# cp2k/dbcsr

Measured on AMD Instinct MI355X. Metric: block-sparse multiply GFLOP/s (fp64), higher is better.
Workload: dtype f64; 1 GPU; config2_32768_23x23_fill10_fp64; M=32768, c_nblks=2030625, nproducts=29207882, k_passes=1, parallelism=1 GPU

## Files before the change

dbcsr_amd/csrc/mm_choose.h:

```cpp
#ifndef DBCSR_AMD_MM_CHOOSE_H
#define DBCSR_AMD_MM_CHOOSE_H

#include <algorithm>
#include <cstddef>
#include <cstdint>
#include <cstdio>

namespace dbcsr_amd {

#define DBCSR_AMD_HOT_SIZES(X) \
  X(9) X(10) X(11) X(12) X(13) X(14) X(15) X(16) X(17) X(18) X(19) X(20) X(21) X(22) X(23) X(24) X(25) X(26) X(27) X(28) X(29) X(30) X(31) X(32)
#define DBCSR_AMD_DMA_SIZES(X) X(13) X(16) X(23) X(32)
#define DBCSR_AMD_F32_DIRECT_SIZES(X) X(16) X(24) X(32)
#define DBCSR_AMD_MID_SHAPES(X)                                                                             \
  X(6, 8) X(6, 9) X(6, 10) X(6, 11) X(6, 12)                                                                \
  X(7, 9) X(7, 10) X(7, 11) X(7, 12)                                                                        \
  X(8, 6) X(8, 8) X(8, 9) X(8, 10) X(8, 11) X(8, 12)                                                        \
  X(9, 6) X(9, 7) X(9, 8) X(9, 9) X(9, 10) X(9, 11) X(9, 12)                                                \
  X(10, 6) X(10, 7) X(10, 8) X(10, 9) X(10, 10) X(10, 11) X(10, 12)                                         \
  X(11, 6) X(11, 7) X(11, 8) X(11, 9) X(11, 10) X(11, 11) X(11, 12)                                         \
  X(12, 6) X(12, 7) X(12, 8) X(12, 9) X(12, 10) X(12, 11) X(12, 12)

#define DBCSR_AMD_IS_(S_) || s == S_
static inline bool hot_f64_has(int m, int n, int k) { const int s = m; return m == n && m == k && (false DBCSR_AMD_HOT_SIZES(DBCSR_AMD_IS_)); }
// ... 232 lines not shown
  c.variant = (lab.dbg & ~32) ? 1 : lab.hot_variant;
  if (hot_allowed && hot_f64_has(hm, hn, hk)) return pick(Family::f64_hot, per_wave, dbg_flags, "mm_numeric_f64_hot<%d,%d,%d>", hm, hn, hk);
  if (sw.use_pipe == 1 || (sw.use_pipe < 0 && f.nproducts < 6 * nblk && f.nproducts > nblk + nblk / 2)) {
    c.group = sw.pipe_g;
    c.lds_bytes = 4 * wave_bytes + (size_t)lab.lds_pad;
    return pick(Family::f64_pipe, (unsigned)((npos + 4 * (int64_t)c.group - 1) / (4 * (int64_t)c.group)), skip, "mm_numeric_f64_pipe<%d>", c.maxt);
  }
  return pick(Family::f64_lds, lds_grid, dbg_flags, "mm_numeric_f64_lds<%d>", c.maxt);
}

struct SymbolicSizes {
  int nbr = 0, nbk = 0, nbc = 0;
  int64_t a_nblks = 0, b_nblks = 0;
  bool filtering = false, retain = false;
  int forced = 0;
};

struct SymbolicChoice {
  bool sparse_guess = false;
  bool bitmap_rows = false;
  bool grid_kernels = false, rows_kernels = false;
};

static inline SymbolicChoice choose_symbolic_pattern(const SymbolicSizes& s) {
  SymbolicChoice c;
  const double prod_est = (double)s.a_nblks * ((double)s.b_nblks / (double)std::max(s.nbk, 1));
  c.sparse_guess = s.forced == 3 || (s.forced == 0 && s.nbr >= 2048 && prod_est < 0.6 * (double)s.nbr * (double)s.nbc);
  c.bitmap_rows = s.filtering && c.sparse_guess && !s.retain;
  return c;
}

static inline SymbolicChoice choose_symbolic_count(const SymbolicSizes& s, SymbolicChoice c, int64_t c_nblks) {
  const int nJ = (s.nbc + 63) / 64;
  c.grid_kernels = s.filtering || (((int64_t)s.nbr * nJ * 64 <= 256 * std::max<int64_t>(c_nblks, 1)) && s.forced != 1);
  c.rows_kernels = s.forced == 3 || (s.forced == 0 && s.nbr >= 2048 && 10 * c_nblks < 6 * (int64_t)s.nbr * s.nbc);
  if (c.rows_kernels) c.grid_kernels = false;
  return c;
}

static inline void choose_panels(int W, int64_t b_bytes_est, int64_t panel_bytes, int* NP_out, int* PW_out) {
  int NP = (int)std::min<int64_t>((b_bytes_est + panel_bytes - 1) / panel_bytes, (int64_t)W);
  if (NP < 1) NP = 1;
  const int PW = (W + NP - 1) / NP;
  *NP_out = (W + PW - 1) / PW;
  *PW_out = PW;
}

static inline int64_t panel_bytes_of_mb(long long mb) { return (int64_t)std::max<long long>(mb, 1) << 20; }

}
#endif
```

dbcsr_amd/csrc/mm_engine.hip:

```cpp
#include <hip/hip_runtime.h>

#include <cstdio>
#include <cstdlib>
#include <cstring>
#include <algorithm>
#include <new>
#include <vector>

#include "../../include/dbcsr_amd_mm.h"
#include "common.h"
#include "smm_core.h"
#include "mm_types.h"
#include "mm_complex.h"
#include "mm_jit.h"

#include "mm_workspace.h"
#include "mm_symbolic.h"
#include "mm_numeric_f64.h"
#include "mm_numeric_f64_big.h"
#include "mm_numeric_f64_small.h"
#include "mm_mid.h"
#include "mm_numeric_f32.h"
#include "mm_numeric_z64.h"
#include "mm_aux.h"
// ... 23 lines not shown
#include "mm_engine_plan.h"
#ifdef DBCSR_AMD_EXPERIMENTS
#include "mm_engine_lab.h"
#endif


static int build_product_lists(Engine* E, bool reuse, const dbcsr_amd_bcsr* a, const dbcsr_amd_bcsr* b, const dbcsr_amd_bcsr* c_in, dbcsr_amd_bcsr* c_out,
                               hipStream_t st) {
  const int nbr = E->facts.nbr, W = E->W, nbc = b->nblkcols, nJ = (nbc + 63) / 64;
  const int64_t nblk = E->facts.c_nblks;
  const uint32_t* cin_bm = E->have_cin ? E->cin_bm.p : nullptr;
  const int* cin_pre = E->have_cin ? E->cin_pre.p : nullptr;
  if (reuse) {
    ACC_CHECK(hipMemcpyAsync(c_out->col_i, E->plan_c_col_i.p, sizeof(int32_t) * (size_t)nblk, hipMemcpyDeviceToDevice, st));
    ACC_CHECK(hipMemcpyAsync(c_out->blk_p, E->plan_c_blk_p.p, sizeof(int64_t) * (size_t)nblk, hipMemcpyDeviceToDevice, st));
  } else if (E->rows_kernels) {
    if (E->tmp_i32.ensure((size_t)nblk + 1)) return -1;
    ACC_CHECK(hipMemsetAsync(E->tmp_i32.p, 0, sizeof(int) * (size_t)nblk, st));
    hipLaunchKernelGGL(fill_products_rows, grid_for((int64_t)nbr * 64), dim3(256), 0, st, a->row_p, a->col_i, a->blk_p, a->col_blk_size, b->row_p,
                       b->col_i, b->blk_p, E->c_bm.p, E->c_pre.p, c_out->row_p, E->prod_start.p, nbr, W, E->tmp_i32.p, E->entries.p, E->filter);
    hipLaunchKernelGGL(finish_descs_grid, grid_for((int64_t)nbr * nJ * 64), dim3(256), 0, st, c_in->row_p, c_in->blk_p, c_out->row_blk_size,
                       c_out->col_blk_size, cin_bm, cin_pre, E->c_bm.p, E->c_pre.p, c_out->row_p, E->c_blk_p_ws.p, E->prod_start.p,
                       E->prod_cnt.p, nbr, W, nJ, c_out->col_i, c_out->blk_p, E->descs.p);
  } else if (E->grid_kernels) {
    hipLaunchKernelGGL(fill_products_grid, grid_for((int64_t)nbr * nJ * 64), dim3(256), 0, st, a->row_p, a->col_i, a->blk_p, b->row_p,
                       b->blk_p, c_in->row_p, c_in->blk_p, a->row_blk_size, a->col_blk_size, b->col_blk_size, E->b_bm.p, E->b_pre.p,
                       cin_bm, cin_pre, E->c_bm.p, E->c_pre.p, c_out->row_p, E->prod_start.p, E->c_blk_p_ws.p, nbr, nbc, W, nJ, c_out->col_i,
                       c_out->blk_p, E->descs.p, E->entries.p, E->filter);
  } else {
    hipLaunchKernelGGL(fill_products, grid_for((int64_t)nbr * W), dim3(256), 0, st, a->row_p, a->col_i, a->blk_p, b->row_p, b->blk_p,
// ... 244 lines not shown
  if (E->b_bm.ensure((size_t)nbk * W + 1) || E->b_pre.ensure((size_t)nbk * W + 1) || E->c_bm.ensure((size_t)nbr * W + 1) ||
      E->c_pre.ensure((size_t)nbr * W + 1) || E->row_nnz.ensure((size_t)nbr + 1) || E->dev_scalars.ensure(16))
    return -1;
  if (E->have_cin && (E->cin_bm.ensure((size_t)nbr * W + 1) || E->cin_pre.ensure((size_t)nbr * W + 1))) return -1;
  ACC_CHECK(hipMemsetAsync(E->dev_scalars.p, 0, 16 * sizeof(unsigned long long), st));
  {
    static const int init[6] = {0, -0x7fffffff, 0, -0x7fffffff, 0, -0x7fffffff};
    ACC_CHECK(hipMemcpyAsync(E->dev_scalars.p + 4, init, sizeof(init), hipMemcpyHostToDevice, st));
  }
  if (nbr == 0 || nbc == 0) {
    ACC_CHECK(hipMemsetAsync(c_out_row_p, 0, sizeof(int32_t) * ((size_t)nbr + 1), st));
    ACC_CHECK(hipStreamSynchronize(st));
    counts->c_nblks = counts->c_nze = counts->nproducts = counts->flop = 0;
    E->facts.c_nblks = 0;
    E->facts.nproducts = 0;
    E->grid_kernels = E->rows_kernels = false;
    E->facts.cls_mode = false;
    E->sym_bitmap = -1;
    E->sym_NP = E->sym_PW = E->sym_rowp_chunks = 0;
    E->valid = true;
    return 0;
  }
  ACC_CHECK(hipMemsetAsync(E->b_bm.p, 0, sizeof(uint32_t) * (size_t)nbk * W, st));
  if (nbk > 0) {
    hipLaunchKernelGGL(bitmap_from_index, grid_for((int64_t)nbk * 64), dim3(256), 0, st, b->row_p, b->col_i, nbk, W, E->b_bm.p);
    hipLaunchKernelGGL(row_prefix, grid_for((int64_t)nbk * 64), dim3(256), 0, st, E->b_bm.p, nbk, W, E->b_pre.p, (int*)nullptr);
  }
  if (E->have_cin) {
    ACC_CHECK(hipMemsetAsync(E->cin_bm.p, 0, sizeof(uint32_t) * (size_t)nbr * W, st));
    hipLaunchKernelGGL(bitmap_from_index, grid_for((int64_t)nbr * 64), dim3(256), 0, st, c_in->row_p, c_in->col_i, nbr, W,
                       E->cin_bm.p);
// ... 11 lines not shown
    } else if (datatype == dbcsr_type_complex_8) {
      hipLaunchKernelGGL((bcsr_block_norms<z64>), grid_for((int64_t)nbr * sa * 64), dim3(256), 0, st, a->row_p, a->col_i, a->blk_p,
                         static_cast<const z64*>(a->data), a->row_blk_size, a->col_blk_size, nbr, sa, 1.0, E->a_norms.p, (double*)nullptr);
      hipLaunchKernelGGL((bcsr_block_norms<z64>), grid_for((int64_t)nbk * sb * 64), dim3(256), 0, st, b->row_p, b->col_i, b->blk_p,
                         static_cast<const z64*>(b->data), b->row_blk_size, b->col_blk_size, nbk, sb, alpha, E->b_norms.p, (double*)nullptr);
    } else {
      hipLaunchKernelGGL((bcsr_block_norms<float>), grid_for((int64_t)nbr * sa * 64), dim3(256), 0, st, a->row_p, a->col_i, a->blk_p,
                         static_cast<const float*>(a->data), a->row_blk_size, a->col_blk_size, nbr, sa, 1.0, E->a_norms.p, (double*)nullptr);
      hipLaunchKernelGGL((bcsr_block_norms<float>), grid_for((int64_t)nbk * sb * 64), dim3(256), 0, st, b->row_p, b->col_i, b->blk_p,
                         static_cast<const float*>(b->data), b->row_blk_size, b->col_blk_size, nbk, sb, alpha, E->b_norms.p, (double*)nullptr);
    }
    E->filter = FilterArgs{E->a_norms.p, E->b_norms.p, (float)filter_eps};
  }
  SymbolicSizes sizes;
  sizes.nbr = nbr, sizes.nbk = nbk, sizes.nbc = nbc, sizes.a_nblks = a->nblks, sizes.b_nblks = b->nblks;
  sizes.filtering = filtering, sizes.retain = retain_sparsity != 0, sizes.forced = E->force_symbolic;
  SymbolicChoice sym = choose_symbolic_pattern(sizes);
  if (sym.bitmap_rows) {
    if (E->have_cin)
      ACC_CHECK(hipMemcpyAsync(E->c_bm.p, E->cin_bm.p, sizeof(uint32_t) * (size_t)nbr * W, hipMemcpyDeviceToDevice, st));
    else
      ACC_CHECK(hipMemsetAsync(E->c_bm.p, 0, sizeof(uint32_t) * (size_t)nbr * W, st));
    hipLaunchKernelGGL(c_bitmap_rows_filtered, grid_for((int64_t)nbr * 64), dim3(256), 0, st, a->row_p, a->col_i, b->row_p, b->col_i, nbr, W,
                       E->facts.canonical_c, E->filter, E->c_bm.p);
  } else if (filtering)
    hipLaunchKernelGGL(c_bitmap_filtered, grid_for((int64_t)nbr * ((nbc + 63) / 64) * 64), dim3(256), 0, st, a->row_p, a->col_i, b->row_p,
                       E->b_bm.p, E->b_pre.p, E->have_cin ? E->cin_bm.p : (const uint32_t*)nullptr, nbr, nbc, W, (nbc + 63) / 64,
                       retain_sparsity ? 1 : 0, E->facts.canonical_c, E->filter, E->c_bm.p);
  else
    hipLaunchKernelGGL(c_bitmap, grid_for((int64_t)nbr * W), dim3(256), 0, st, a->row_p, a->col_i, E->b_bm.p,
                       E->have_cin ? E->cin_bm.p : (const uint32_t*)nullptr, nbr, W, retain_sparsity ? 1 : 0, E->facts.canonical_c, E->c_bm.p);
// ... 64 lines not shown
  } else {
  hipLaunchKernelGGL(order_count, grid_for(nkeys), dim3(256), 0, st, E->c_pre.p, E->row_nnz.p, nbr, W, PW, NP, NG, RG, E->order_cnt.p);
  if (exclusive_scan<int64_t>(E, E->order_cnt.p, nkeys, E->order_base.p, nullptr, false, st)) return -1;
  hipLaunchKernelGGL(order_len, dim3(1), dim3(1), 0, st, E->order_base.p, c_nblks, NP, NG, dsc + 7);
  }
  if (E->prod_cnt.ensure((size_t)c_nblks + 1) || E->blk_nze.ensure((size_t)c_nblks + 1) || E->prod_start.ensure((size_t)c_nblks + 1) ||
      E->c_blk_p_ws.ensure((size_t)c_nblks + 1))
    return -1;
  const int nJ = (nbc + 63) / 64;
  sym = choose_symbolic_count(sizes, sym, c_nblks);
  E->grid_kernels = sym.grid_kernels;
  E->rows_kernels = sym.rows_kernels;
  E->sym_bitmap = sym.bitmap_rows ? 2 : (filtering ? 1 : 0);
  E->sym_NP = NP, E->sym_PW = PW;
  E->sym_rowp_chunks = (int)(((int64_t)nbr + kScanChunk - 1) / kScanChunk);
  if (E->rows_kernels) {
    ACC_CHECK(hipMemsetAsync(E->prod_cnt.p, 0, sizeof(int) * (size_t)c_nblks, st));
    hipLaunchKernelGGL(block_sizes_rows, grid_for((int64_t)nbr * W), dim3(256), 0, st, E->c_bm.p, E->c_pre.p, c_out_row_p, a->row_blk_size,
                       b->col_blk_size, nbr, W, E->blk_nze.p);
    hipLaunchKernelGGL(count_products_rows, grid_for((int64_t)nbr * 64), dim3(256), 0, st, a->row_p, a->col_i, a->row_blk_size, a->col_blk_size,
                       b->col_blk_size, b->row_p, b->col_i, E->c_bm.p, E->c_pre.p, c_out_row_p, nbr, W, E->prod_cnt.p, E->dev_scalars.p + 3,
                       E->filter);
  } else if (E->grid_kernels)
    hipLaunchKernelGGL(count_products_grid, grid_for((int64_t)nbr * nJ * 64), dim3(256), 0, st, a->row_p, a->col_i, a->row_blk_size,
                       a->col_blk_size, b->col_blk_size, E->b_bm.p, E->c_bm.p, E->c_pre.p, c_out_row_p, nbr, nbc, W, nJ,
                       E->prod_cnt.p, E->blk_nze.p, E->dev_scalars.p + 3, b->row_p, E->b_pre.p, E->filter);
  else
    hipLaunchKernelGGL(count_products, grid_for((int64_t)nbr * W), dim3(256), 0, st, a->row_p, a->col_i, a->row_blk_size,
                       a->col_blk_size, b->col_blk_size, E->b_bm.p, E->c_bm.p, E->c_pre.p, c_out_row_p, nbr, W, E->prod_cnt.p,
                       E->blk_nze.p, E->dev_scalars.p + 3);
  if (exclusive_scan<int64_t>(E, E->prod_cnt.p, c_nblks, E->prod_start.p, dsc + 2, false, st)) return -1;
  if (exclusive_scan<int64_t>(E, E->blk_nze.p, c_nblks, E->c_blk_p_ws.p, dsc + 1, false, st)) return -1;
  ACC_CHECK(hipMemcpyAsync(E->host_scalars, dsc, 8 * sizeof(int64_t), hipMemcpyDeviceToHost, st));
  ACC_CHECK(hipStreamSynchronize(st));
  E->facts.order_len = E->host_scalars[7];
  if (E->facts.cls_mode) {
    for (int c = 0; c < kNumClasses; ++c) {
      E->cls_len[c] = E->cls_host_lens[c];
      E->cls_off[c] = E->cls_host_lens[kNumClasses + c];
    }
    const int64_t total = E->cls_host_lens[2 * kNumClasses];
    E->facts.order_len = total / 8;
    if (E->order.ensure((size_t)total + 64)) return -1;
    if (total > 0) {
      ACC_CHECK(hipMemsetAsync(E->order.p, 0xff, sizeof(int) * ((size_t)total + 64), st));
      hipLaunchKernelGGL(order_fill_cls, grid_for((int64_t)nbr * W), dim3(256), 0, st, E->c_bm.p, E->c_pre.p, c_out_row_p, E->cls_row.p,
// ... 121 lines not shown
```

dbcsr_amd/csrc/mm_engine_env.h:

```cpp
#ifndef DBCSR_AMD_MM_ENGINE_ENV_H
#define DBCSR_AMD_MM_ENGINE_ENV_H

static void engine_read_env(Engine* E) {
  if (const char* k = getenv("DBCSR_AMD_MM_KERNEL")) {
    E->sw.use_lds = strcmp(k, "direct") != 0;
    E->sw.use_pipe = strcmp(k, "pipe") == 0 ? 1 : (strcmp(k, "lds1") == 0 ? 0 : -1);
#ifdef DBCSR_AMD_EXPERIMENTS
    if (strncmp(k, "dma", 3) == 0 && k[3] >= '2' && k[3] <= '4') E->lab.dma_stages = k[3] - '0';
#endif
  }
  if (const char* k = getenv("DBCSR_AMD_MM_PIPE_G")) E->sw.pipe_g = std::max(1, atoi(k));
  if (const char* k = getenv("DBCSR_AMD_MM_CLASSES")) E->sw.use_classes = atoi(k);
  if (const char* k = getenv("DBCSR_AMD_MM_WORK")) E->sw.use_work = atoi(k);
  if (const char* k = getenv("DBCSR_AMD_MM_WG_WAVES")) {
    const int w = atoi(k);
    if (w == 1 || w == 2 || w == 4) E->sw.wg_waves = w;
  }
  if (const char* k = getenv("DBCSR_AMD_MM_PLAN")) E->use_plan = atoi(k);
  if (const char* k = getenv("DBCSR_AMD_MM_HOT")) E->sw.use_hot = atoi(k);
  if (const char* k = getenv("DBCSR_AMD_MM_TINY")) E->sw.use_tiny = atoi(k);
  if (const char* k = getenv("DBCSR_AMD_MM_SMALL")) E->sw.use_small = atoi(k);
  if (const char* k = getenv("DBCSR_AMD_MM_SMALL_G")) E->sw.small_group = std::min(64, std::max(0, atoi(k)));
  if (const char* k = getenv("DBCSR_AMD_MM_F32_DIRECT")) E->sw.f32_direct = atoi(k);
  if (const char* k = getenv("DBCSR_AMD_MM_BIG")) E->sw.use_big = atoi(k);
  if (const char* k = getenv("DBCSR_AMD_MM_MID")) E->sw.use_mid = atoi(k);
  if (const char* k = getenv("DBCSR_AMD_MM_SYMBOLIC")) {
    E->force_symbolic = strcmp(k, "word") == 0 ? 1 : (strcmp(k, "grid") == 0 ? 2 : (strcmp(k, "rows") == 0 ? 3 : 0));
  }
  if (const char* k = getenv("DBCSR_AMD_MM_PANEL_MB")) E->panel_bytes = panel_bytes_of_mb(atoll(k));
#ifdef DBCSR_AMD_EXPERIMENTS
  if (const char* k = getenv("DBCSR_AMD_MM_F32_GROUP")) {
    const int r = atoi(k);
    E->lab.f32_group = (r >= 2 && r <= 4) ? r : (r < 0 ? -1 : 0);
  }
  if (const char* k = getenv("DBCSR_AMD_MM_F64_GROUP")) E->lab.f64_group = atoi(k);
  if (const char* k = getenv("DBCSR_AMD_MM_GROUP_PANEL_MB")) E->ls.group_panel_bytes = panel_bytes_of_mb(atoll(k));
  if (const char* k = getenv("DBCSR_AMD_MM_CLASS_G")) {
    const int g = atoi(k);
    E->lab.class_g = (g == 2 || g == 4 || g == 8) ? g : 1;
  }
  if (const char* k = getenv("DBCSR_AMD_MM_DBG")) E->lab.dbg = atoi(k);
  if (const char* k = getenv("DBCSR_AMD_ALG_COLSUMS")) E->ls.alg_col_variant = atoi(k);
  if (const char* k = getenv("DBCSR_AMD_MULTIVEC_WAVES")) E->ls.multivec_waves = atoi(k);
// ... 28 lines not shown
```

dbcsr_amd/csrc/mm_engine_ops.h:

```cpp
#ifndef DBCSR_AMD_MM_ENGINE_OPS_H
#define DBCSR_AMD_MM_ENGINE_OPS_H

static int init_c_any(void* handle, libsmm_acc_data_t datatype, double beta, double beta_im, const dbcsr_amd_bcsr* c_in, dbcsr_amd_bcsr* c_out,
                      void* stream) {
  Engine* E = static_cast<Engine*>(handle);
  if (E) E->plan_numeric = false;
  if (!E || !E->valid || !c_in || !c_out) {
    fprintf(stderr, "dbcsr_amd_mm_init_c: no valid symbolic phase for this handle\n");
    return -1;
  }
  if (datatype != dbcsr_type_real_8 && datatype != dbcsr_type_real_4 && datatype != dbcsr_type_complex_8) return -10;
  hipStream_t st = stream_of(stream);
  const int nbr = E->facts.nbr, W = E->W;
  const int64_t nblk = E->facts.c_nblks;
  engine_writes_values(E);
  c_out->nblks = nblk;
  if (nblk == 0) return 0;
  if (E->descs.ensure((size_t)nblk + 1)) return -1;
  hipLaunchKernelGGL(emit_index, grid_for((int64_t)nbr * W), dim3(256), 0, st, c_in->row_p, c_in->blk_p, c_out->row_blk_size,
                     c_out->col_blk_size, E->have_cin ? E->cin_bm.p : (const uint32_t*)nullptr,
                     E->have_cin ? E->cin_pre.p : (const int*)nullptr, E->c_bm.p, E->c_pre.p, c_out->row_p, E->c_blk_p_ws.p, nbr, W,
                     c_out->col_i, c_out->blk_p, E->descs.p);
  if (datatype == dbcsr_type_real_8)
    hipLaunchKernelGGL((init_c_blocks<double>), grid_for(nblk * 64), dim3(256), 0, st, E->descs.p, nblk,
// ... 467 lines not shown
const char* dbcsr_amd_mm_last_kernel(void* handle) {
  Engine* E = static_cast<Engine*>(handle);
  return E ? E->last_kernel : "";
}

const char* dbcsr_amd_mm_last_symbolic(void* handle) {
  Engine* E = static_cast<Engine*>(handle);
  if (!E) return "";
  static const char* const bitmap[] = {"none", "plain", "filtered", "rows_filtered"};
  snprintf(E->last_symbolic, sizeof E->last_symbolic, "bitmap=%s count=%s W=%d NP=%d PW=%d classes=%d rowp_chunks=%d plan=%s",
           bitmap[std::min(std::max(E->sym_bitmap, -1), 2) + 1], E->sym_bitmap < 0 ? "none" : (E->rows_kernels ? "rows" : (E->grid_kernels ? "grid" : "word")),
           E->W, E->sym_NP, E->sym_PW, E->facts.cls_mode ? 1 : 0, E->sym_rowp_chunks, E->plan_hit ? "hit" : "miss");
  return E->last_symbolic;
}

int dbcsr_amd_mm_expect_filter(void* handle, double eps) {
  Engine* E = static_cast<Engine*>(handle);
  if (!E || !(eps >= 0.0)) return -1;
  E->drop_pending = eps * eps;
  return 0;
}

int dbcsr_amd_mm_trust_plan(void* handle, int on) {
  Engine* E = static_cast<Engine*>(handle);
  if (!E) return -1;
  E->plan_trusted = on != 0;
  return 0;
}

int dbcsr_amd_mm_plan_stats(void* handle, int64_t* reused, int64_t* built) {
// ... 57 lines not shown
```

dbcsr_amd/csrc/mm_engine_state.h:

```cpp
#ifndef DBCSR_AMD_MM_ENGINE_STATE_H
#define DBCSR_AMD_MM_ENGINE_STATE_H

struct PlanSegs {
  const int32_t* a[12];
  const int32_t* b[12];
  long long n[12];
  int nseg;
};
__global__ void __launch_bounds__(256) plan_compare(PlanSegs S, int* __restrict__ differs) {
  const long long stride = (long long)gridDim.x * blockDim.x;
  bool bad = false;
  for (int g = 0; g < S.nseg; ++g)
    for (long long i = (long long)blockIdx.x * blockDim.x + threadIdx.x; i < S.n[g]; i += stride) bad |= S.a[g][i] != S.b[g][i];
  if (__ballot(bad) && (threadIdx.x & 63) == 0) atomicOr(differs, 1);
}

#ifdef DBCSR_AMD_EXPERIMENTS
struct LabState {
  int group_R = 0;
  bool group_built = false, b_monotone = false;
  int64_t group_panel_bytes = 0;
  DevBuf<int> groups, group_flag, group_cnt;
  DevBuf<GWork> group_work;
  DevBuf<GEntry> group_entries;
// ... 46 lines not shown
  DevBuf<unsigned char> cls_row, cls_col;
  DevBuf<int> cls_vpos, cls_vrow;
  DevBuf<uint32_t> cls_col_bm;
  DevBuf<int64_t> cls_lens;
  int* cls_host_hist = nullptr;
  int64_t* cls_host_lens = nullptr;
  hipEvent_t ev[3] = {nullptr, nullptr, nullptr};
  hipStream_t side_stream[3] = {nullptr, nullptr, nullptr};
  hipEvent_t fork_ev = nullptr, join_ev[3] = {nullptr, nullptr, nullptr};

  SizeFacts facts;
  int W = 0;
  bool have_cin = false, valid = false;
  bool rows_kernels = false;
  bool grid_kernels = false;
  int sym_bitmap = -1, sym_NP = 0, sym_PW = 0, sym_rowp_chunks = 0;
  char last_symbolic[160] = "";
  int64_t cls_len[kNumClasses] = {0}, cls_off[kNumClasses] = {0};
  FilterArgs filter = {nullptr, nullptr, 0.0f};
  double drop_pending = 0.0;
  bool work_built = false;

  const void* norms_data = nullptr;
  int64_t norms_nblks = 0;
  double unwritten_below = 0.0;
  char last_kernel[96] = "";
  bool timed = false;
  int64_t flt_nblks = 0;
  int64_t flt_new_nblks = -1;
  int filter_in_place = 0;
// ... 54 lines not shown
    const void* rs = nullptr;
    const void* cs = nullptr;
    uint64_t stamp = 0;
    int nbr = 0, nbc = 0;
    int64_t nblks = 0, nslots = 0;
    int64_t nze = -1;
  };
  static constexpr int kCsrLens = 8;
  CsrLen csr_len[kCsrLens];
  int csr_len_next = 0;

  Switches sw;
  LabSwitches lab;
  int use_plan = 1;
  int force_symbolic = 0;
  int64_t panel_bytes = 256ll << 20;

  bool plan_saved = false, plan_hit = false, plan_numeric = false;
  int plan_dims[3] = {0, 0, 0}, plan_retain = 0, plan_canonical = 0, plan_datatype = 0;
  int64_t plan_nblks[3] = {0, 0, 0};
  bool plan_trusted = false;
  const void* plan_ptrs[12] = {nullptr};
  uint64_t plan_stamps[3] = {0, 0, 0};
  DevBuf<int32_t> plan_words, plan_c_col_i;
  DevBuf<int64_t> plan_c_blk_p;
  DevBuf<int> plan_flag;
  int* plan_host_flag = nullptr;
  dbcsr_amd_mm_counts plan_counts = {0, 0, 0, 0};
  long long plan_hits = 0, plan_misses = 0;

// ... 47 lines not shown
```

dbcsr_amd/csrc/mm_symbolic.h:

```cpp
#ifndef DBCSR_AMD_MM_SYMBOLIC_H
#define DBCSR_AMD_MM_SYMBOLIC_H
#include "mm_epilogue.h"

namespace dbcsr_amd {


__global__ void __launch_bounds__(256) bitmap_from_index(const int* __restrict__ row_p, const int* __restrict__ col_i, int nbr, int W,
                                                         uint32_t* __restrict__ bm) {
  const int lane = threadIdx.x & 63;
  const int row = (blockIdx.x * blockDim.x + threadIdx.x) >> 6;
  if (row >= nbr) return;
  for (int b = row_p[row] + lane; b < row_p[row + 1]; b += 64) {
    const int j = col_i[b];
    atomicOr(&bm[(size_t)row * W + (j >> 5)], 1u << (j & 31));
  }
}

__device__ __forceinline__ uint32_t canonical_bits(int i, int w) {
  const uint32_t even = (i & 1) ? 0xAAAAAAAAu : 0x55555555u;
  const int d = i - 32 * w;
  const uint32_t upper = d <= 0 ? 0xFFFFFFFFu : (d >= 32 ? 0u : ~((1u << d) - 1u));
  return (even & upper) | (~even & ~upper);
}

// ... 458 lines not shown
  d.c_off = c_blk_p_ws[cb];
  d.cin_off = -1;
  if (cin_bm) {
    const uint32_t cinw = cin_bm[t];
    if ((cinw >> bit) & 1u) d.cin_off = cin_blk_p[cin_row_p[i] + cin_pre[t] + __popc(cinw & below)];
  }
  d.prod_start = prod_start[cb];
  d.prod_cnt = prod_cnt[cb];
  d.m = (int16_t)rs[i];
  d.n = (int16_t)cs[j];
  descs[cb] = d;
  c_col_i[cb] = j;
  c_blk_p[cb] = d.c_off;
}

__global__ void __launch_bounds__(256)
emit_index(const int* __restrict__ cin_row_p, const int64_t* __restrict__ cin_blk_p, const int* __restrict__ rs,
           const int* __restrict__ cs, const uint32_t* __restrict__ cin_bm, const int* __restrict__ cin_pre,
           const uint32_t* __restrict__ c_bm, const int* __restrict__ c_pre, const int* __restrict__ c_row_p,
           const int64_t* __restrict__ c_blk_p_ws, int nbr, int W, int* __restrict__ c_col_i, int64_t* __restrict__ c_blk_p,
           Desc* __restrict__ descs) {
  const int64_t t = (int64_t)blockIdx.x * blockDim.x + threadIdx.x;
  if (t >= (int64_t)nbr * W) return;
  const int i = (int)(t / W), w = (int)(t % W);
  uint32_t v = c_bm[t];
  if (!v) return;
  int cb = c_row_p[i] + c_pre[t];
  const uint32_t cinw = cin_bm ? cin_bm[t] : 0u;
  while (v) {
    const int bit = __ffs(v) - 1;
// ... 230 lines not shown
```

dbcsr_amd/lib.py:

```python
import ctypes as C
import os

_HERE = os.path.dirname(os.path.abspath(__file__))
_LIB = None
_LIB_LAB = None

dbcsr_type_real_4 = 1
dbcsr_type_real_8 = 3
dbcsr_type_complex_4 = 5
dbcsr_type_complex_8 = 7

ACC_SYMBOLS = [
    "c_dbcsr_acc_init", "c_dbcsr_acc_finalize", "c_dbcsr_acc_clear_errors", "c_dbcsr_acc_get_ndevices",
    "c_dbcsr_acc_set_active_device", "c_dbcsr_acc_device_synchronize", "c_dbcsr_acc_stream_priority_range",
    "c_dbcsr_acc_stream_create", "c_dbcsr_acc_stream_destroy", "c_dbcsr_acc_stream_sync", "c_dbcsr_acc_stream_wait_event",
    "c_dbcsr_acc_event_create", "c_dbcsr_acc_event_destroy", "c_dbcsr_acc_event_record", "c_dbcsr_acc_event_query",
    "c_dbcsr_acc_event_synchronize", "c_dbcsr_acc_dev_mem_allocate", "c_dbcsr_acc_dev_mem_deallocate",
    "c_dbcsr_acc_dev_mem_set_ptr", "c_dbcsr_acc_host_mem_allocate", "c_dbcsr_acc_host_mem_deallocate",
    "c_dbcsr_acc_memcpy_h2d", "c_dbcsr_acc_memcpy_d2h", "c_dbcsr_acc_memcpy_d2d", "c_dbcsr_acc_memset_zero",
    "c_dbcsr_acc_dev_mem_info", "c_dbcsr_timeset", "c_dbcsr_timestop",
]
LIBSMM_SYMBOLS = [
    "libsmm_acc_init", "libsmm_acc_finalize", "libsmm_acc_is_thread_safe", "libsmm_acc_transpose", "libsmm_acc_process",
    "c_calculate_norms", "libsmm_acc_gpu_warp_size",
]
MM_SYMBOLS = [
    "dbcsr_amd_mm_create", "dbcsr_amd_mm_destroy", "dbcsr_amd_mm_symbolic", "dbcsr_amd_mm_numeric", "dbcsr_amd_bcsr_transpose",
    "dbcsr_amd_bcsr_checksum", "dbcsr_amd_bcsr_fill_random", "dbcsr_amd_mm_kernel_name", "dbcsr_amd_mm_last_kernel", "dbcsr_amd_mm_last_symbolic", "dbcsr_amd_fabric_probe", "dbcsr_amd_mm_plan_stats", "dbcsr_amd_mm_trust_plan", "dbcsr_amd_mm_expect_filter", "dbcsr_amd_mm_stats", "dbcsr_amd_mm_timing", "dbcsr_amd_mm_init_c", "dbcsr_amd_bcsr_fill_random_dist",
    "dbcsr_amd_mm_symbolic_filtered", "dbcsr_amd_bcsr_filter_count", "dbcsr_amd_bcsr_filter_apply",
    "dbcsr_amd_bcsr_crop_count", "dbcsr_amd_bcsr_crop_apply", "dbcsr_amd_bcsr_scale_window",
    "dbcsr_amd_multiply", "dbcsr_amd_bcsr_release", "dbcsr_amd_bcsr_desymmetrize_count", "dbcsr_amd_bcsr_desymmetrize_apply",
    "dbcsr_amd_bcsr_twin_count", "dbcsr_amd_bcsr_twin_apply", "dbcsr_amd_mm_set_canonical_product", "dbcsr_amd_multiply_symmetric_c",
    "dbcsr_amd_bcsr_desymmetrized", "dbcsr_amd_smm_last_kernel", "dbcsr_amd_multiply_symmetric_c_klimits",
    "dbcsr_amd_bcsr_filter_apply_index", "dbcsr_amd_mm_set_filter_in_place",
    "dbcsr_amd_mm_numeric_z", "dbcsr_amd_mm_init_c_z", "dbcsr_amd_bcsr_scale_window_z", "dbcsr_amd_bcsr_transpose_conj", "dbcsr_amd_multiply_z",
    "dbcsr_amd_multiply_symmetric_c_z",
    "dbcsr_amd_bcsr_add_count", "dbcsr_amd_bcsr_add_apply", "dbcsr_amd_bcsr_diag_count", "dbcsr_amd_bcsr_diag_fill", "dbcsr_amd_bcsr_diag_shift",
    "dbcsr_amd_bcsr_trace", "dbcsr_amd_bcsr_dot", "dbcsr_amd_bcsr_norm2",
    "dbcsr_amd_bcsr_maxabs", "dbcsr_amd_bcsr_row_sums", "dbcsr_amd_bcsr_col_sums", "dbcsr_amd_bcsr_gershgorin", "dbcsr_amd_bcsr_get_diag",
    "dbcsr_amd_bcsr_set_diag", "dbcsr_amd_bcsr_scale_by_vector", "dbcsr_amd_bcsr_matvec", "dbcsr_amd_bcsr_multivec",
    "dbcsr_amd_bcsr_rank_update",
    "dbcsr_amd_bcsr_block_diag_count", "dbcsr_amd_bcsr_block_diag_apply", "dbcsr_amd_bcsr_block_diag_invert",
    "dbcsr_amd_bcsr_block_diag_multiply",
# ... 113 lines not shown
    L.dbcsr_amd_bcsr_desymmetrized.argtypes = [vp, i32, BP, i32, BP, vp]
    L.dbcsr_amd_multiply_symmetric_c.argtypes = [vp, C.c_char, C.c_char, i32, C.c_double, BP, BP, C.c_double, BP, i32, i32, C.c_double, BP,
                                                 C.POINTER(i64), vp]
    L.dbcsr_amd_mm_stats.argtypes = [vp, C.POINTER(MnkStat), i32, C.POINTER(i32), vp]
    L.dbcsr_amd_comm_available.argtypes = []
    L.dbcsr_amd_comm_unique_id.argtypes = [C.c_char_p]
    L.dbcsr_amd_comm_create.argtypes = [C.POINTER(vp), C.c_char_p, i32, i32]
    L.dbcsr_amd_comm_destroy.argtypes = [vp]
    L.dbcsr_amd_comm_rank.argtypes = [vp, C.POINTER(i32), C.POINTER(i32)]
    L.dbcsr_amd_comm_exchange.argtypes = [vp, C.POINTER(CommOp), i32, C.POINTER(CommOp), i32, vp]
    L.dbcsr_amd_comm_allgather.argtypes = [vp, vp, vp, i64, vp]
    L.dbcsr_amd_mm_last_kernel.argtypes = [vp]
    L.dbcsr_amd_mm_last_kernel.restype = C.c_char_p
    L.dbcsr_amd_mm_last_symbolic.argtypes = [vp]
    L.dbcsr_amd_mm_last_symbolic.restype = C.c_char_p
    L.dbcsr_amd_smm_last_kernel.argtypes = []
    L.dbcsr_amd_smm_last_kernel.restype = C.c_char_p
    L.dbcsr_amd_fabric_probe.argtypes = [C.POINTER(C.c_double), C.POINTER(C.c_double)]
    L.dbcsr_amd_mm_plan_stats.argtypes = [vp, C.POINTER(i64), C.POINTER(i64)]
    L.dbcsr_amd_mm_trust_plan.argtypes = [vp, C.c_int]
    L.dbcsr_amd_mm_expect_filter.argtypes = [vp, C.c_double]
    L.dbcsr_amd_mm_expect_filter.restype = C.c_int
    Z = C.POINTER(C.c_double)
    L.dbcsr_amd_mm_numeric_z.argtypes = [vp, Z, BP, BP, Z, BP, BP, vp]
    L.dbcsr_amd_mm_init_c_z.argtypes = [vp, Z, BP, BP, vp]
    L.dbcsr_amd_bcsr_scale_window_z.argtypes = [vp, BP, Z, i64, i64, i64, i64, vp]
    L.dbcsr_amd_bcsr_transpose_conj.argtypes = [vp, i32, BP, BP, vp]
    L.dbcsr_amd_multiply_z.argtypes = [vp, C.c_char, C.c_char, Z, BP, BP, Z, BP, C.POINTER(i64), i32, C.c_double, BP, C.POINTER(i64), vp]
    L.dbcsr_amd_multiply_symmetric_c_z.argtypes = [vp, C.c_char, C.c_char, Z, BP, BP, Z, BP, i32, i64, i64, i32, C.c_double, BP, C.POINTER(i64), vp]
    L.dbcsr_amd_bcsr_add_count.argtypes = [vp, BP, BP, i32, vp, C.POINTER(i64), C.POINTER(i64), C.POINTER(i32), vp]
# ... 46 lines not shown
```

dbcsr_amd/multiply.py:

```python
import ctypes as C
import math
import os

import torch

from . import lib as _lib
from .matrix import DbcsrMatrix, StreamHandle, symmetry_kind

dbcsr_no_transpose = "N"
dbcsr_transpose = "T"
dbcsr_conjugate_transpose = "C"


def _z(x):
    x = complex(x)
    return (C.c_double * 2)(x.real, x.imag)


class MultiplyEngine:

    def __init__(self, lab=None):
        self.lab = _lib.want_lab() if lab is None else bool(lab)
        self.L = _lib.load_library(self.lab)
        self.h = C.c_void_p()
# ... 72 lines not shown
        for (m, n, k), (cnt, fl) in sorted(tot.items(), key=lambda kv: -kv[1][1]):
            print(" flops %5d x %5d x %5d %20d       0.0%%      0.0%%    100.0%%" % (m, n, k, fl), file=f)
        print(" flops total %30.6E       0.0%%      0.0%%    100.0%%" % float(total), file=f)
        print(" matmuls total %28d       0.0%%      0.0%%    100.0%%" % sum(v[0] for v in tot.values()), file=f)
        print(" # multiplications %24d" % self.__dict__.get("stats_multiplications", 0), file=f)
        print(" " + "-" * 79, file=f)

    def last_kernel(self):
        eng = getattr(self, "_last_pass_engine", None) if getattr(self, "last_kchunks", 1) > 1 else None
        v = self.L.dbcsr_amd_mm_last_kernel((eng or self).h)
        return v.decode() if v else ""

    def last_symbolic(self):
        v = self.L.dbcsr_amd_mm_last_symbolic(self.h)
        return v.decode() if v else ""

    def plan_stats(self):
        a, b = C.c_int64(), C.c_int64()
        if self.L.dbcsr_amd_mm_plan_stats(self.h, C.byref(a), C.byref(b)) != 0:
            raise RuntimeError("dbcsr_amd_mm_plan_stats failed")
        return a.value, b.value

    def trust_plan(self, on=True):
        if self.L.dbcsr_amd_mm_trust_plan(self.h, 1 if on else 0) != 0:
            raise RuntimeError("dbcsr_amd_mm_trust_plan failed")

    def tile_stats(self):
        a, b = C.c_int(), C.c_int()
        rc = self.L.dbcsr_amd_mm_tile_stats(self.h, C.byref(a), C.byref(b))
        if rc < 0:
# ... 410 lines not shown
```

include/dbcsr_amd_mm.h:

```cpp
#ifndef DBCSR_AMD_MM_H
#define DBCSR_AMD_MM_H

#include <stdint.h>

#include "dbcsr_acc_libsmm.h"

#if defined(__cplusplus)
extern "C" {
#endif

typedef struct dbcsr_amd_bcsr {
  int32_t nblkrows, nblkcols;
  const int32_t* row_blk_size;
  const int32_t* col_blk_size;
  int32_t* row_p;
  int32_t* col_i;
  int64_t* blk_p;
  void* data;
  int64_t nblks;
  uint64_t index_stamp;
} dbcsr_amd_bcsr;

typedef struct dbcsr_amd_mm_counts {
  int64_t c_nblks;
// ... 73 lines not shown
int dbcsr_amd_multiply_symmetric_c(void* handle, char transa, char transb, libsmm_acc_data_t datatype, double alpha,
  const dbcsr_amd_bcsr* matrix_a, const dbcsr_amd_bcsr* matrix_b, double beta, const dbcsr_amd_bcsr* matrix_c, int kind,
  int retain_sparsity, double filter_eps, dbcsr_amd_bcsr* c_out, int64_t* flop, void* stream);
int dbcsr_amd_multiply_symmetric_c_klimits(void* handle, char transa, char transb, libsmm_acc_data_t datatype, double alpha,
  const dbcsr_amd_bcsr* matrix_a, const dbcsr_amd_bcsr* matrix_b, double beta, const dbcsr_amd_bcsr* matrix_c, int kind,
  int64_t first_k, int64_t last_k, int retain_sparsity, double filter_eps, dbcsr_amd_bcsr* c_out, int64_t* flop, void* stream);
int dbcsr_amd_multiply_symmetric_c_z(void* handle, char transa, char transb, const double alpha[2], const dbcsr_amd_bcsr* matrix_a,
  const dbcsr_amd_bcsr* matrix_b, const double beta[2], const dbcsr_amd_bcsr* matrix_c, int kind, int64_t first_k, int64_t last_k,
  int retain_sparsity, double filter_eps, dbcsr_amd_bcsr* c_out, int64_t* flop, void* stream);

int dbcsr_amd_mm_stats(void* handle, dbcsr_amd_mnk_stat* out, int max_entries, int* n_entries, void* stream);

const char* dbcsr_amd_mm_kernel_name(libsmm_acc_data_t datatype);
const char* dbcsr_amd_mm_last_kernel(void* handle);
const char* dbcsr_amd_mm_last_symbolic(void* handle);
const char* dbcsr_amd_smm_last_kernel(void);

int dbcsr_amd_mm_trust_plan(void* handle, int on);

int dbcsr_amd_mm_expect_filter(void* handle, double eps);
int dbcsr_amd_mm_plan_stats(void* handle, int64_t* reused, int64_t* built);

int dbcsr_amd_bcsr_add_count(void* handle, const dbcsr_amd_bcsr* a, const dbcsr_amd_bcsr* b, int beta_is_zero, int32_t* dst_row_p, int64_t* nblks,
  int64_t* nze, int* same_pattern, void* stream);
int dbcsr_amd_bcsr_add_apply(void* handle, libsmm_acc_data_t datatype, const double alpha[2], const dbcsr_amd_bcsr* a, const double beta[2],
  const dbcsr_amd_bcsr* b, dbcsr_amd_bcsr* dst, void* stream);
int dbcsr_amd_bcsr_diag_count(void* handle, const dbcsr_amd_bcsr* m, int32_t* dst_row_p, int32_t* dst_col_i, int64_t* dst_blk_p, int64_t* nblks,
  int64_t* nze, void* stream);
int dbcsr_amd_bcsr_diag_fill(void* handle, libsmm_acc_data_t datatype, const double alpha[2], dbcsr_amd_bcsr* dst, void* stream);
int dbcsr_amd_bcsr_diag_shift(void* handle, libsmm_acc_data_t datatype, dbcsr_amd_bcsr* m, const double alpha[2], void* stream);
// ... 78 lines not shown
```

Before: 38140 GFLOP/s.

## Add row-wise LDS counting-sort symbolic path for product list construction

Adds a new symbolic path that builds per-row product lists with one workgroup per C block row. Each wave keeps per-column counters in LDS and runs a count sweep, a block scan and then a fill sweep, writing descriptors and entries in column order without global per-block count arrays. It replaces the global prod_cnt atomics and scan over all C blocks with a per-row product count and scan, and is enabled by default when there is no filtering, retain or canonical mode and A has at least one block per row. The cost is LDS sized to 4*nbc ints per workgroup, which limits occupancy for wide matrices, plus an extra pass over B rows.

```diff
diff --git a/dbcsr_amd/csrc/mm_choose.h b/dbcsr_amd/csrc/mm_choose.h
--- a/dbcsr_amd/csrc/mm_choose.h
+++ b/dbcsr_amd/csrc/mm_choose.h
@@ -270,6 +270,7 @@
   int64_t a_nblks = 0, b_nblks = 0;
   bool filtering = false, retain = false;
   int forced = 0;
+  bool canonical = false;
 };
 
 struct SymbolicChoice {
@@ -294,6 +295,17 @@
   return c;
 }
 
+constexpr int kListsWaves = 4;
+constexpr int kListsMaxCols = (65536 - 64) / (kListsWaves * (int)sizeof(int32_t));
+static inline bool lists_legal(const SymbolicSizes& s) {
+  return !s.filtering && !s.retain && !s.canonical && s.nbc <= kListsMaxCols && (int64_t)s.nbk * (int64_t)s.nbc <= 0x7fffffffll;
+}
+static inline bool choose_symbolic_lists(const SymbolicSizes& s, const SymbolicChoice& c, int64_t c_nblks, int lists_switch) {
+  if (lists_switch == 0 || !lists_legal(s) || c_nblks <= 0) return false;
+  if (lists_switch == 1) return true;
+  return s.forced == 0 && !c.rows_kernels && s.a_nblks >= (int64_t)s.nbr;
+}
+
 static inline void choose_panels(int W, int64_t b_bytes_est, int64_t panel_bytes, int* NP_out, int* PW_out) {
   int NP = (int)std::min<int64_t>((b_bytes_est + panel_bytes - 1) / panel_bytes, (int64_t)W);
   if (NP < 1) NP = 1;
diff --git a/dbcsr_amd/csrc/mm_engine.hip b/dbcsr_amd/csrc/mm_engine.hip
--- a/dbcsr_amd/csrc/mm_engine.hip
+++ b/dbcsr_amd/csrc/mm_engine.hip
@@ -61,6 +61,10 @@
   if (reuse) {
     ACC_CHECK(hipMemcpyAsync(c_out->col_i, E->plan_c_col_i.p, sizeof(int32_t) * (size_t)nblk, hipMemcpyDeviceToDevice, st));
     ACC_CHECK(hipMemcpyAsync(c_out->blk_p, E->plan_c_blk_p.p, sizeof(int64_t) * (size_t)nblk, hipMemcpyDeviceToDevice, st));
+  } else if (E->lists_rows) {
+    hipLaunchKernelGGL(list_products_rows_lds, dim3((unsigned)nbr), dim3(256), lists_lds_bytes(nbc), st, a->row_p, a->col_i, a->blk_p, b->row_p, b->col_i,
+                       b->blk_p, c_in->row_p, c_in->blk_p, a->row_blk_size, a->col_blk_size, b->col_blk_size, cin_bm, cin_pre, E->c_bm.p, E->c_pre.p,
+                       c_out->row_p, E->row_prod_start.p, E->c_blk_p_ws.p, nbc, W, c_out->col_i, c_out->blk_p, E->descs.p, E->entries.p);
   } else if (E->rows_kernels) {
     if (E->tmp_i32.ensure((size_t)nblk + 1)) return -1;
     ACC_CHECK(hipMemsetAsync(E->tmp_i32.p, 0, sizeof(int) * (size_t)nblk, st));
@@ -335,7 +339,7 @@
     counts->c_nblks = counts->c_nze = counts->nproducts = counts->flop = 0;
     E->facts.c_nblks = 0;
     E->facts.nproducts = 0;
-    E->grid_kernels = E->rows_kernels = false;
+    E->grid_kernels = E->rows_kernels = E->lists_rows = false;
     E->facts.cls_mode = false;
     E->sym_bitmap = -1;
     E->sym_NP = E->sym_PW = E->sym_rowp_chunks = 0;
@@ -377,7 +381,7 @@
   }
   SymbolicSizes sizes;
   sizes.nbr = nbr, sizes.nbk = nbk, sizes.nbc = nbc, sizes.a_nblks = a->nblks, sizes.b_nblks = b->nblks;
-  sizes.filtering = filtering, sizes.retain = retain_sparsity != 0, sizes.forced = E->force_symbolic;
+  sizes.filtering = filtering, sizes.retain = retain_sparsity != 0, sizes.forced = E->force_symbolic, sizes.canonical = E->facts.canonical_c != 0;
   SymbolicChoice sym = choose_symbolic_pattern(sizes);
   if (sym.bitmap_rows) {
     if (E->have_cin)
@@ -472,6 +476,17 @@
   E->sym_bitmap = sym.bitmap_rows ? 2 : (filtering ? 1 : 0);
   E->sym_NP = NP, E->sym_PW = PW;
   E->sym_rowp_chunks = (int)(((int64_t)nbr + kScanChunk - 1) / kScanChunk);
+  E->lists_rows = choose_symbolic_lists(sizes, sym, c_nblks, E->use_lists);
+  if (E->lists_rows) {
+    if (E->row_prod.ensure((size_t)nbr + 1) || E->row_prod_start.ensure((size_t)nbr + 2) || E->b_row_n.ensure((size_t)nbk + 1)) return -1;
+    hipLaunchKernelGGL(block_sizes_rows, grid_for((int64_t)nbr * W), dim3(256), 0, st, E->c_bm.p, E->c_pre.p, c_out_row_p, a->row_blk_size,
+                       b->col_blk_size, nbr, W, E->blk_nze.p);
+    if (nbk > 0)
+      hipLaunchKernelGGL(b_row_col_sizes, grid_for((int64_t)nbk * 64), dim3(256), 0, st, b->row_p, b->col_i, b->col_blk_size, nbk, E->b_row_n.p);
+    hipLaunchKernelGGL(row_products, grid_for((int64_t)nbr * 64), dim3(256), 0, st, a->row_p, a->col_i, a->row_blk_size, a->col_blk_size, b->row_p,
+                       E->b_row_n.p, nbr, E->row_prod.p, E->dev_scalars.p + 3);
+    if (exclusive_scan<int64_t>(E, E->row_prod.p, nbr, E->row_prod_start.p, dsc + 2, true, st)) return -1;
+  } else {
   if (E->rows_kernels) {
     ACC_CHECK(hipMemsetAsync(E->prod_cnt.p, 0, sizeof(int) * (size_t)c_nblks, st));
     hipLaunchKernelGGL(block_sizes_rows, grid_for((int64_t)nbr * W), dim3(256), 0, st, E->c_bm.p, E->c_pre.p, c_out_row_p, a->row_blk_size,
@@ -488,6 +503,7 @@
                        a->col_blk_size, b->col_blk_size, E->b_bm.p, E->c_bm.p, E->c_pre.p, c_out_row_p, nbr, W, E->prod_cnt.p,
                        E->blk_nze.p, E->dev_scalars.p + 3);
   if (exclusive_scan<int64_t>(E, E->prod_cnt.p, c_nblks, E->prod_start.p, dsc + 2, false, st)) return -1;
+  }
   if (exclusive_scan<int64_t>(E, E->blk_nze.p, c_nblks, E->c_blk_p_ws.p, dsc + 1, false, st)) return -1;
   ACC_CHECK(hipMemcpyAsync(E->host_scalars, dsc, 8 * sizeof(int64_t), hipMemcpyDeviceToHost, st));
   ACC_CHECK(hipStreamSynchronize(st));
diff --git a/dbcsr_amd/csrc/mm_engine_env.h b/dbcsr_amd/csrc/mm_engine_env.h
--- a/dbcsr_amd/csrc/mm_engine_env.h
+++ b/dbcsr_amd/csrc/mm_engine_env.h
@@ -27,6 +27,7 @@
   if (const char* k = getenv("DBCSR_AMD_MM_SYMBOLIC")) {
     E->force_symbolic = strcmp(k, "word") == 0 ? 1 : (strcmp(k, "grid") == 0 ? 2 : (strcmp(k, "rows") == 0 ? 3 : 0));
   }
+  if (const char* k = getenv("DBCSR_AMD_MM_LISTS")) E->use_lists = atoi(k) == 0 ? 0 : (atoi(k) == 1 ? 1 : -1);
   if (const char* k = getenv("DBCSR_AMD_MM_PANEL_MB")) E->panel_bytes = panel_bytes_of_mb(atoll(k));
 #ifdef DBCSR_AMD_EXPERIMENTS
   if (const char* k = getenv("DBCSR_AMD_MM_F32_GROUP")) {
diff --git a/dbcsr_amd/csrc/mm_engine_ops.h b/dbcsr_amd/csrc/mm_engine_ops.h
--- a/dbcsr_amd/csrc/mm_engine_ops.h
+++ b/dbcsr_amd/csrc/mm_engine_ops.h
@@ -505,6 +505,11 @@
   return E->last_symbolic;
 }
 
+int dbcsr_amd_mm_last_lists(void* handle) {
+  Engine* E = static_cast<Engine*>(handle);
+  return E ? (E->valid && E->facts.c_nblks > 0 && E->lists_rows ? 1 : 0) : -1;
+}
+
 int dbcsr_amd_mm_expect_filter(void* handle, double eps) {
   Engine* E = static_cast<Engine*>(handle);
   if (!E || !(eps >= 0.0)) return -1;
diff --git a/dbcsr_amd/csrc/mm_engine_state.h b/dbcsr_amd/csrc/mm_engine_state.h
--- a/dbcsr_amd/csrc/mm_engine_state.h
+++ b/dbcsr_amd/csrc/mm_engine_state.h
@@ -84,6 +84,10 @@
   bool have_cin = false, valid = false;
   bool rows_kernels = false;
   bool grid_kernels = false;
+  bool lists_rows = false;
+  DevBuf<int> row_prod;
+  DevBuf<int64_t> row_prod_start;
+  DevBuf<long long> b_row_n;
   int sym_bitmap = -1, sym_NP = 0, sym_PW = 0, sym_rowp_chunks = 0;
   char last_symbolic[160] = "";
   int64_t cls_len[kNumClasses] = {0}, cls_off[kNumClasses] = {0};
@@ -168,6 +172,7 @@
   LabSwitches lab;
   int use_plan = 1;
   int force_symbolic = 0;
+  int use_lists = -1;
   int64_t panel_bytes = 256ll << 20;
 
   bool plan_saved = false, plan_hit = false, plan_numeric = false;
diff --git a/dbcsr_amd/csrc/mm_symbolic.h b/dbcsr_amd/csrc/mm_symbolic.h
--- a/dbcsr_amd/csrc/mm_symbolic.h
+++ b/dbcsr_amd/csrc/mm_symbolic.h
@@ -496,6 +496,185 @@
   c_blk_p[cb] = d.c_off;
 }
 
+
+__global__ void __launch_bounds__(256) b_row_col_sizes(const int* __restrict__ b_row_p, const int* __restrict__ b_col_i, const int* __restrict__ cs,
+                                                       int nbk, long long* __restrict__ b_row_n) {
+  const int lane = threadIdx.x & 63;
+  const int k = (int)(((int64_t)blockIdx.x * blockDim.x + threadIdx.x) >> 6);
+  if (k >= nbk) return;
+  long long s = 0;
+  for (int bb = b_row_p[k] + lane; bb < b_row_p[k + 1]; bb += 64) s += cs[b_col_i[bb]];
+  s = wave_sum(s);
+  if (lane == 0) b_row_n[k] = s;
+}
+
+__global__ void __launch_bounds__(256) row_products(const int* __restrict__ a_row_p, const int* __restrict__ a_col_i, const int* __restrict__ rs,
+                                                    const int* __restrict__ ks, const int* __restrict__ b_row_p, const long long* __restrict__ b_row_n,
+                                                    int nbr, int* __restrict__ row_prod, unsigned long long* __restrict__ flop_out) {
+  const int lane = threadIdx.x & 63;
+  const int i = (int)(((int64_t)blockIdx.x * blockDim.x + threadIdx.x) >> 6);
+  unsigned long long flop = 0;
+  if (i < nbr) {
+    int cnt = 0;
+    unsigned long long kn = 0;
+    for (int ab = a_row_p[i] + lane; ab < a_row_p[i + 1]; ab += 64) {
+      const int k = a_col_i[ab];
+      cnt += b_row_p[k + 1] - b_row_p[k];
+      kn += (unsigned long long)ks[k] * (unsigned long long)b_row_n[k];
+    }
+    cnt = wave_sum(cnt);
+    flop = 2ull * (unsigned long long)rs[i] * wave_sum(kn);
+    if (lane == 0) row_prod[i] = cnt;
+  }
+  __shared__ unsigned long long red[4];
+  if (lane == 0) red[threadIdx.x >> 6] = flop;
+  __syncthreads();
+  if (threadIdx.x == 0) {
+    const unsigned long long t = red[0] + red[1] + red[2] + red[3];
+    if (t) atomicAdd(flop_out, t);
+  }
+}
+
+constexpr int kListsDepth = 4;
+template <bool FILL>
+__device__ __forceinline__ void lists_sweep(int q0, int q1, int lane, const int* __restrict__ a_col_i, const int64_t* __restrict__ a_blk_p,
+                                            const int* __restrict__ ks, const int* __restrict__ b_row_p, const int* __restrict__ b_col_i,
+                                            const int64_t* __restrict__ b_blk_p, int* cnt, Entry* __restrict__ row_entries) {
+  for (int base = q0; base < q1; base += 64) {
+    const int n = min(64, q1 - base);
+    int my_b0 = 0, my_b1 = 0, my_kk = 0;
+    long long my_a = 0;
+    if (lane < n) {
+      const int k = a_col_i[base + lane];
+      my_b0 = b_row_p[k];
+      my_b1 = b_row_p[k + 1];
+      if (FILL) my_kk = ks[k], my_a = a_blk_p[base + lane];
+    }
+    int t = 0, off = -64, b0 = __builtin_amdgcn_readlane(my_b0, 0), b1 = __builtin_amdgcn_readlane(my_b1, 0);
+    auto next = [&]() {
+      off += 64;
+      while (t < n && b0 + off >= b1) {
+        ++t, off = 0;
+        if (t < n) b0 = __builtin_amdgcn_readlane(my_b0, t), b1 = __builtin_amdgcn_readlane(my_b1, t);
+      }
+    };
+    constexpr int D = kListsDepth;
+    int j_c[D], t_c[D], j_n[D], t_n[D];
+    long long bo_c[D], bo_n[D];
+    auto fetch = [&](int& j, long long& bo, int& tp) {
+      next();
+      tp = t, j = -1, bo = 0;
+      if (t < n && b0 + off + lane < b1) {
+        j = b_col_i[b0 + off + lane];
+        if (FILL) bo = b_blk_p[b0 + off + lane];
+      }
+    };
+#pragma unroll
+    for (int d = 0; d < D; ++d) fetch(j_c[d], bo_c[d], t_c[d]);
+    while (t_c[0] < n) {
+#pragma unroll
+      for (int d = 0; d < D; ++d) fetch(j_n[d], bo_n[d], t_n[d]);
+#pragma unroll
+      for (int d = 0; d < D; ++d) {
+        if (t_c[d] < n) {
+          if (FILL) {
+            const uint32_t a_lo = (uint32_t)__builtin_amdgcn_readlane((int)(uint32_t)my_a, t_c[d]);
+            const uint32_t a_hi = (uint32_t)__builtin_amdgcn_readlane((int)(uint32_t)((unsigned long long)my_a >> 32), t_c[d]);
+            const long long a_off = (long long)(((unsigned long long)a_hi << 32) | a_lo);
+            const int kk = __builtin_amdgcn_readlane(my_kk, t_c[d]);
+            if (j_c[d] >= 0) row_entries[atomicAdd(&cnt[j_c[d]], 1)] = Entry::make(a_off, bo_c[d], kk);
+          } else if (j_c[d] >= 0) {
+            atomicAdd(&cnt[j_c[d]], 1);
+          }
+        }
+      }
+#pragma unroll
+      for (int d = 0; d < D; ++d) j_c[d] = j_n[d], bo_c[d] = bo_n[d], t_c[d] = t_n[d];
+    }
+  }
+}
+
+__device__ __forceinline__ int lists_block_scan(int v, int* scratch, int* total) {
+  const int lane = threadIdx.x & 63, w = threadIdx.x >> 6;
+  int inc = v;
+#pragma unroll
+  for (int o = 1; o < 64; o <<= 1) {
+    const int u = __shfl_up(inc, o, 64);
+    if (lane >= o) inc += u;
+  }
+  if (lane == 63) scratch[w] = inc;
+  __syncthreads();
+  int woff = 0, tot = 0;
+#pragma unroll
+  for (int q = 0; q < 4; ++q) {
+    if (q < w) woff += scratch[q];
+    tot += scratch[q];
+  }
+  __syncthreads();
+  *total = tot;
+  return woff + inc - v;
+}
+
+static inline size_t lists_lds_bytes(int nbc) { return ((size_t)4 * (size_t)nbc + 16) * sizeof(int); }
+
+__global__ void __launch_bounds__(256)
+list_products_rows_lds(const int* __restrict__ a_row_p, const int* __restrict__ a_col_i, const int64_t* __restrict__ a_blk_p,
+                       const int* __restrict__ b_row_p, const int* __restrict__ b_col_i, const int64_t* __restrict__ b_blk_p,
+                       const int* __restrict__ cin_row_p, const int64_t* __restrict__ cin_blk_p, const int* __restrict__ rs,
+                       const int* __restrict__ ks, const int* __restrict__ cs, const uint32_t* __restrict__ cin_bm,
+                       const int* __restrict__ cin_pre, const uint32_t* __restrict__ c_bm, const int* __restrict__ c_pre,
+                       const int* __restrict__ c_row_p, const int64_t* __restrict__ row_prod_start, const int64_t* __restrict__ c_blk_p_ws, int nbc,
+                       int W, int* __restrict__ c_col_i, int64_t* __restrict__ c_blk_p, Desc* __restrict__ descs, Entry* __restrict__ entries) {
+  extern __shared__ int lists_lds[];
+  int* scratch = lists_lds + (size_t)4 * nbc;
+  const int i = blockIdx.x, lane = threadIdx.x & 63, w = threadIdx.x >> 6;
+  for (int t = threadIdx.x; t < 4 * nbc; t += 256) lists_lds[t] = 0;
+  __syncthreads();
+  const int a0 = a_row_p[i], na = a_row_p[i + 1] - a0;
+  const int q0 = a0 + (int)((int64_t)na * w / 4), q1 = a0 + (int)((int64_t)na * (w + 1) / 4);
+  int* cnt = lists_lds + (size_t)w * nbc;
+  const int64_t row_start = row_prod_start[i];
+  lists_sweep<false>(q0, q1, lane, a_col_i, a_blk_p, ks, b_row_p, b_col_i, b_blk_p, cnt, nullptr);
+  __syncthreads();
+  int carry = 0;
+  const int m = rs[i], cb0 = c_row_p[i];
+  for (int jt = 0; jt < nbc; jt += 256) {
+    const int j = jt + (int)threadIdx.x;
+    int c0 = 0, c1 = 0, c2 = 0, c3 = 0;
+    if (j < nbc) c0 = lists_lds[j], c1 = lists_lds[nbc + j], c2 = lists_lds[2 * nbc + j], c3 = lists_lds[3 * nbc + j];
+    const int tot = c0 + c1 + c2 + c3;
+    int tile_total;
+    const int first = carry + lists_block_scan(tot, scratch, &tile_total);
+    carry += tile_total;
+    if (j < nbc) {
+      lists_lds[j] = first, lists_lds[nbc + j] = first + c0, lists_lds[2 * nbc + j] = first + c0 + c1, lists_lds[3 * nbc + j] = first + c0 + c1 + c2;
+      const int wj = j >> 5, bit = j & 31;
+      const size_t t = (size_t)i * W + wj;
+      const uint32_t cw = c_bm[t];
+      if ((cw >> bit) & 1u) {
+        const uint32_t below = (1u << bit) - 1u;
+        const int cb = cb0 + c_pre[t] + __popc(cw & below);
+        Desc d;
+        d.c_off = c_blk_p_ws[cb];
+        d.cin_off = -1;
+        if (cin_bm) {
+          const uint32_t cinw = cin_bm[t];
+          if ((cinw >> bit) & 1u) d.cin_off = cin_blk_p[cin_row_p[i] + cin_pre[t] + __popc(cinw & below)];
+        }
+        d.prod_start = row_start + first;
+        d.prod_cnt = tot;
+        d.m = (int16_t)m;
+        d.n = (int16_t)cs[j];
+        descs[cb] = d;
+        c_col_i[cb] = j;
+        c_blk_p[cb] = d.c_off;
+      }
+    }
+  }
+  __syncthreads();
+  lists_sweep<true>(q0, q1, lane, a_col_i, a_blk_p, ks, b_row_p, b_col_i, b_blk_p, cnt, entries + row_start);
+}
+
 __global__ void __launch_bounds__(256)
 emit_index(const int* __restrict__ cin_row_p, const int64_t* __restrict__ cin_blk_p, const int* __restrict__ rs,
            const int* __restrict__ cs, const uint32_t* __restrict__ cin_bm, const int* __restrict__ cin_pre,
diff --git a/dbcsr_amd/lib.py b/dbcsr_amd/lib.py
--- a/dbcsr_amd/lib.py
+++ b/dbcsr_amd/lib.py
@@ -26,7 +26,7 @@
 ]
 MM_SYMBOLS = [
     "dbcsr_amd_mm_create", "dbcsr_amd_mm_destroy", "dbcsr_amd_mm_symbolic", "dbcsr_amd_mm_numeric", "dbcsr_amd_bcsr_transpose",
-    "dbcsr_amd_bcsr_checksum", "dbcsr_amd_bcsr_fill_random", "dbcsr_amd_mm_kernel_name", "dbcsr_amd_mm_last_kernel", "dbcsr_amd_mm_last_symbolic", "dbcsr_amd_fabric_probe", "dbcsr_amd_mm_plan_stats", "dbcsr_amd_mm_trust_plan", "dbcsr_amd_mm_expect_filter", "dbcsr_amd_mm_stats", "dbcsr_amd_mm_timing", "dbcsr_amd_mm_init_c", "dbcsr_amd_bcsr_fill_random_dist",
+    "dbcsr_amd_bcsr_checksum", "dbcsr_amd_bcsr_fill_random", "dbcsr_amd_mm_kernel_name", "dbcsr_amd_mm_last_kernel", "dbcsr_amd_mm_last_symbolic", "dbcsr_amd_mm_last_lists", "dbcsr_amd_fabric_probe", "dbcsr_amd_mm_plan_stats", "dbcsr_amd_mm_trust_plan", "dbcsr_amd_mm_expect_filter", "dbcsr_amd_mm_stats", "dbcsr_amd_mm_timing", "dbcsr_amd_mm_init_c", "dbcsr_amd_bcsr_fill_random_dist",
     "dbcsr_amd_mm_symbolic_filtered", "dbcsr_amd_bcsr_filter_count", "dbcsr_amd_bcsr_filter_apply",
     "dbcsr_amd_bcsr_crop_count", "dbcsr_amd_bcsr_crop_apply", "dbcsr_amd_bcsr_scale_window",
     "dbcsr_amd_multiply", "dbcsr_amd_bcsr_release", "dbcsr_amd_bcsr_desymmetrize_count", "dbcsr_amd_bcsr_desymmetrize_apply",
@@ -170,6 +170,8 @@
     L.dbcsr_amd_mm_last_kernel.restype = C.c_char_p
     L.dbcsr_amd_mm_last_symbolic.argtypes = [vp]
     L.dbcsr_amd_mm_last_symbolic.restype = C.c_char_p
+    L.dbcsr_amd_mm_last_lists.argtypes = [vp]
+    L.dbcsr_amd_mm_last_lists.restype = C.c_int
     L.dbcsr_amd_smm_last_kernel.argtypes = []
     L.dbcsr_amd_smm_last_kernel.restype = C.c_char_p
     L.dbcsr_amd_fabric_probe.argtypes = [C.POINTER(C.c_double), C.POINTER(C.c_double)]
diff --git a/dbcsr_amd/multiply.py b/dbcsr_amd/multiply.py
--- a/dbcsr_amd/multiply.py
+++ b/dbcsr_amd/multiply.py
@@ -110,6 +110,9 @@
     def last_symbolic(self):
         v = self.L.dbcsr_amd_mm_last_symbolic(self.h)
         return v.decode() if v else ""
+
+    def last_lists(self):
+        return self.L.dbcsr_amd_mm_last_lists(self.h) == 1
 
     def plan_stats(self):
         a, b = C.c_int64(), C.c_int64()
diff --git a/include/dbcsr_amd_mm.h b/include/dbcsr_amd_mm.h
--- a/include/dbcsr_amd_mm.h
+++ b/include/dbcsr_amd_mm.h
@@ -111,6 +111,7 @@
 const char* dbcsr_amd_mm_kernel_name(libsmm_acc_data_t datatype);
 const char* dbcsr_amd_mm_last_kernel(void* handle);
 const char* dbcsr_amd_mm_last_symbolic(void* handle);
+int dbcsr_amd_mm_last_lists(void* handle);
 const char* dbcsr_amd_smm_last_kernel(void);
 
 int dbcsr_amd_mm_trust_plan(void* handle, int on);
```

Measured after the change: 38100 GFLOP/s. Within noise of the previous version (-0.1%).
